# ysymyth/3D-SDN

Hardware: AMD Instinct MI355X
Metric: rendered-objects/sec (FFD decode + transform + silhouette/normal/depth @384, fwd+bwd) (higher is better)
Workload: dtype f32

## Files before the change

3d-sdn_amd/csrc/raster_fwd.hip:

```cpp
#include <mutex>
#include <type_traits>
#include <vector>

#include "camera_math.h"
#include "raster_math.h"
#include "sdn_common.h"

namespace sdn {

constexpr int TS = 32;
constexpr int NTHR = (TS / 2) * (TS / 2);
constexpr int NWAVE = NTHR / 64;
static_assert(NTHR % 64 == 0 && NTHR >= 2 * TS && TS <= 32, "tile / workgroup geometry (hit queue packs px, py in 5 bits)");
constexpr int QCAP = 512;
constexpr int FREC = 13;
#ifndef SDN_LAB_FLAT_MAX
#define SDN_LAB_FLAT_MAX 256
#endif
constexpr int FLAT_MAX = SDN_LAB_FLAT_MAX;
static_assert(FLAT_MAX >= 1 && FLAT_MAX <= 256, "a batch's stream holds at most 64 * 256 candidates: 14 bits of start, at most 256 passes (the marks are u16, 0xffff = none)");
#ifndef SDN_LAB_HIZ_MIN_LIST
#define SDN_LAB_HIZ_MIN_LIST 257
#endif
constexpr int HIZ_MIN_LIST = SDN_LAB_HIZ_MIN_LIST;
#ifndef SDN_K1_HIZ
#define SDN_K1_HIZ 1
#endif
constexpr uint32_t TB_CULLED = 0x000000FFu;

struct FwdParams {
    const float* faces;
    const float* textures;
    const float* bg;
    float* face_inv;
    int32_t* face_index_map;
    float* weight_map;
    float* depth_map;
    float* rgb_map;
    float* rgb_out;
    float* alpha_out;
    float* depth_out;
    const uint32_t* tilebox;
    const uint4* pixbox;
    const uint32_t* tile_off;
    const uint32_t* tile_list;
    const uint32_t* overflow;
    const uint32_t* tile_order;
    const uint32_t* thin_count;
    const float4* thin_list;
    unsigned long long* counters;
    uint32_t list_cap;
    double eps;
    int ts, bs, nf, S, ntx, flags, bg_per_batch;
    int hiz;
    float near_le, far_f;
};

constexpr float THIN_MARGIN = 4.0f;

__device__ __forceinline__ float face_margin_px(const float f[9], int S)
{
    const float ex0 = f[3] - f[0], ey0 = f[4] - f[1];
    const float ex1 = f[6] - f[0], ey1 = f[7] - f[1];
    const float ex2 = f[6] - f[3], ey2 = f[7] - f[4];
    const float l0 = sqrtf(ex0 * ex0 + ey0 * ey0);
    const float l1 = sqrtf(ex1 * ex1 + ey1 * ey1);
    const float l2 = sqrtf(ex2 * ex2 + ey2 * ey2);
    const float lmax = fmaxf(l0, fmaxf(l1, l2));
    const float perim = l0 + l1 + l2;
    float cmax = fmaxf(fmaxf(fabsf(f[0]), fabsf(f[1])), fmaxf(fabsf(f[3]), fabsf(f[4])));
    cmax = fmaxf(cmax, fmaxf(fabsf(f[6]), fabsf(f[7])));
    const float area2 = fabsf(ex0 * ey1 - ex1 * ey0) - 9.5367432e-7f * lmax * lmax;
    if (!(area2 > 0.0f)) return -1.0f;
    const float delta = 9.5367432e-7f * (1.0f + cmax);
    const float base = 0.004f * fmaxf(1.0f, (float)S * (1.0f / 1024.0f)) + 0.5f * (float)S * delta;
    const float m = base + 0.5f * (float)S * (delta * perim * lmax / area2);
    if (!(m < (float)S)) return -1.0f;
    return m;
}

constexpr int HIST_MAX = 4096;

template <bool K1, bool GATHER>
__global__ __launch_bounds__(256) void k_face_setup(const float* __restrict__ faces, int nf, int S, int ntx,
                                                     float* __restrict__ face_inv, uint32_t* __restrict__ tilebox,
                                                     uint4* __restrict__ pixbox, uint32_t* __restrict__ tile_count,
                                                     uint32_t* __restrict__ thin_count, float4* __restrict__ thin_list,
                                                     const FaceSource G)
{
    __shared__ uint32_t hist[HIST_MAX];
    const int ntiles = ntx * ntx;
    const bool use_lds = ntiles <= HIST_MAX;
    if (use_lds)
        for (int t = threadIdx.x; t < ntiles; t += 256) hist[t] = 0u;
    __syncthreads();
    const int b = blockIdx.y;
    const int t_local = blockIdx.x * 256 + threadIdx.x;
    uint32_t* gcount = tile_count + (size_t)b * ntiles;
    const bool pairs = GATHER && G.fill_back != 0;
    const int nthr = pairs ? G.nf0 : nf;
    float v[3][3], pf[9];
    if constexpr (GATHER) {
        if (t_local < nthr) {
            const int32_t* idx = G.faces_idx + (size_t)b * G.fstride + (size_t)t_local * 3;
#pragma unroll
            for (int k = 0; k < 3; k++) {
                const float* p = G.verts + ((size_t)b * G.nv + idx[k]) * 3;
                v[k][0] = G.flip_x ? p[0] * -1.0f : p[0];
                v[k][1] = p[1];
                v[k][2] = p[2];
            }
            Basis B;
            if (G.mode != 0) B = camera_basis(G.mode, G.eye, G.dir, G.up, b);
            const float wv = G.width ? G.width[b] : 1.0f;
#pragma unroll
            for (int k = 0; k < 3; k++) {
                float o[3];
                project_vertex(v[k], G.mode, B, G.width != nullptr, wv, o);
                pf[3 * k + 0] = o[0];
                pf[3 * k + 1] = o[1];
                pf[3 * k + 2] = o[2];
            }
        }
    }
    if (t_local < nthr)
    for (int rep = 0; rep < (pairs ? 2 : 1); rep++) {
    const int fn_local = t_local + (rep ? G.nf0 : 0);
    const long i = (long)b * nf + fn_local;
    float f[9];
    float nrm[3] = {0.f, 0.f, 0.f};
    if constexpr (GATHER) {
        if (G.normals_out) {
            if (rep)
                face_normal(v[2], v[1], v[0], G.sx, nrm);
            else
                face_normal(v[0], v[1], v[2], G.sx, nrm);
        }
#pragma unroll
        for (int k = 0; k < 3; k++)
#pragma unroll
            for (int d = 0; d < 3; d++) f[3 * k + d] = rep ? pf[3 * (2 - k) + d] : pf[3 * k + d];
    } else {
#pragma unroll
        for (int k = 0; k < 9; k++) f[k] = faces[i * 9 + k];
    }
    float inv[9] = {0, 0, 0, 0, 0, 0, 0, 0, 0};
    uint32_t tb = TB_CULLED;
    uint4 pb = make_uint4(0, 0, 0, 0);
    bool thin = false;
    if constexpr (K1) {
      if (!is_backface(f)) {
        bool finite = true;
// ... 134 lines not shown
            if (G.normals_out) {
                float* o = G.normals_out + i * 3;
                o[0] = nrm[0];
                o[1] = nrm[1];
                o[2] = nrm[2];
            }
        }
    }
    }
    __syncthreads();
    if (use_lds)
        for (int t = threadIdx.x; t < ntiles; t += 256) {
            const uint32_t c = hist[t];
            if (c) atomicAdd(&gcount[t], c);
        }
}

constexpr int ORDER_CLASSES = 64;
__device__ __forceinline__ int order_class(uint32_t entries, bool streams_all_faces)
{
    if (streams_all_faces) return 0;
    const int c = (int)(4.0f * __log2f((float)entries + 1.0f));
    return ORDER_CLASSES - 1 - min(ORDER_CLASSES - 1, c);
}

__global__ __launch_bounds__(256) void k_tile_offsets(const uint32_t* __restrict__ tile_count, int ntiles,
                                                       uint32_t list_cap, uint32_t* __restrict__ tile_off,
                                                       uint32_t* __restrict__ overflow, uint32_t* __restrict__ order_hist)
{
    __shared__ uint32_t wave_tot[4];
    __shared__ uint32_t carry_s;
    __shared__ uint32_t hist[ORDER_CLASSES];
    const int b = blockIdx.x, tid = threadIdx.x;
    if (tid < ORDER_CLASSES) hist[tid] = 0u;
    const uint32_t* cnt = tile_count + (size_t)b * ntiles;
    uint32_t* off = tile_off + (size_t)b * (ntiles + 1);
    if (tid == 0) carry_s = 0u;
    __syncthreads();
    for (int base = 0; base < ntiles; base += 256) {
        const int t = base + tid;
        const uint32_t v = t < ntiles ? cnt[t] : 0u;
        uint32_t incl = v;
#pragma unroll
        for (int d = 1; d < 64; d <<= 1) {
            const uint32_t o = __shfl_up(incl, d, 64);
            if ((tid & 63) >= d) incl += o;
        }
        if ((tid & 63) == 63) wave_tot[tid >> 6] = incl;
        __syncthreads();
        uint32_t wave_off = 0, total = 0;
#pragma unroll
        for (int w = 0; w < 4; w++) {
            const uint32_t x = wave_tot[w];
            if (w < (tid >> 6)) wave_off += x;
            total += x;
        }
        const uint32_t carry = carry_s;
        if (t < ntiles) off[t] = carry + wave_off + incl - v;
        __syncthreads();
        if (tid == 0) carry_s = carry + total;
        __syncthreads();
    }
    if (tid == 0) {
        off[ntiles] = carry_s;
        overflow[b] = carry_s > list_cap ? 1u : 0u;
    }
    const bool streams = carry_s > list_cap;
    for (int t = tid; t < ntiles; t += 256) atomicAdd(&hist[order_class(cnt[t], streams)], 1u);
    __syncthreads();
    if (tid < ORDER_CLASSES && hist[tid]) atomicAdd(&order_hist[tid], hist[tid]);
}

__global__ __launch_bounds__(256) void k_tile_order(const uint32_t* __restrict__ tile_count, int ntiles, int total,
                                                     const uint32_t* __restrict__ overflow,
                                                     const uint32_t* __restrict__ order_hist,
                                                     uint32_t* __restrict__ order_cursor, uint32_t* __restrict__ tile_order)
{
    __shared__ uint32_t base[ORDER_CLASSES];
    const int tid = threadIdx.x;
    if (tid < 64) {
        const uint32_t v = order_hist[tid];
        uint32_t incl = v;
#pragma unroll
        for (int d = 1; d < 64; d <<= 1) {
            const uint32_t o = __shfl_up(incl, d, 64);
            if (tid >= d) incl += o;
        }
        base[tid] = incl - v;
    }
    __shared__ uint32_t lcnt[ORDER_CLASSES], lbase[ORDER_CLASSES];
    if (tid < ORDER_CLASSES) lcnt[tid] = 0u;
    __syncthreads();
    const int g = blockIdx.x * 256 + tid;
    int c = 0;
    uint32_t local = 0;
    if (g < total) {
        c = order_class(tile_count[g], overflow[g / ntiles] != 0u);
        local = atomicAdd(&lcnt[c], 1u);
    }
    __syncthreads();
    if (tid < ORDER_CLASSES && lcnt[tid]) lbase[tid] = base[tid] + atomicAdd(&order_cursor[tid], lcnt[tid]);
    __syncthreads();
    if (g < total) tile_order[lbase[c] + local] = (uint32_t)g;
}

__global__ __launch_bounds__(256) void k_tile_fill(const uint32_t* __restrict__ tilebox, int nf, int ntx,
                                                    const uint32_t* __restrict__ tile_off,
                                                    const uint32_t* __restrict__ overflow, uint32_t list_cap,
                                                    uint32_t* __restrict__ tile_cursor, uint32_t* __restrict__ tile_list)
{
    __shared__ uint32_t cnt[HIST_MAX];
    __shared__ uint32_t base[HIST_MAX];
    const int b = blockIdx.y;
    if (overflow[b]) return;
    const int fn = blockIdx.x * 256 + threadIdx.x;
    const uint32_t v = fn < nf ? tilebox[(size_t)b * nf + fn] : TB_CULLED;
    const int tx0 = (int)(v & 255u), tx1 = (int)((v >> 8) & 255u), ty0 = (int)((v >> 16) & 255u), ty1 = (int)(v >> 24);
    const bool active = tx0 <= tx1;
    const int ntiles = ntx * ntx;
    const uint32_t* off = tile_off + (size_t)b * (ntiles + 1);
    uint32_t* cur = tile_cursor + (size_t)b * ntiles;
    uint32_t* lst = tile_list + (size_t)b * list_cap;
    if (ntiles > HIST_MAX) {
        if (active)
            for (int ty = ty0; ty <= ty1; ty++)
                for (int tx = tx0; tx <= tx1; tx++) {
                    const int tt = ty * ntx + tx;
                    lst[off[tt] + atomicAdd(&cur[tt], 1u)] = (uint32_t)fn;
                }
        return;
    }
    for (int t = threadIdx.x; t < ntiles; t += 256) cnt[t] = 0u;
    __syncthreads();
    if (active)
        for (int ty = ty0; ty <= ty1; ty++)
            for (int tx = tx0; tx <= tx1; tx++) atomicAdd(&cnt[ty * ntx + tx], 1u);
    __syncthreads();
    for (int t = threadIdx.x; t < ntiles; t += 256) {
        const uint32_t c = cnt[t];
        if (c) {
            base[t] = off[t] + atomicAdd(&cur[t], c);
            cnt[t] = 0u;
        }
    }
    __syncthreads();
    if (active)
        for (int ty = ty0; ty <= ty1; ty++)
            for (int tx = tx0; tx <= tx1; tx++) {
                const int tt = ty * ntx + tx;
                lst[base[tt] + atomicAdd(&cnt[tt], 1u)] = (uint32_t)fn;
            }
}

struct PixelResult {
    int fn;
    float w[3];
    float zp;
    float rgb[3];
    float alpha;
};

__device__ __forceinline__ PixelResult shade_pixel(const FwdParams& P, int b, unsigned long long key, int gx, int gy)
{
    PixelResult r;
    const bool want_rgb = (P.flags & SDN_RGB) != 0;
    float bgc[3] = {0.f, 0.f, 0.f};
    if (want_rgb) {
        const float* c = P.bg + (P.bg_per_batch ? 3 * b : 0);
        bgc[0] = c[0];
        bgc[1] = c[1];
        bgc[2] = c[2];
    }
    if (key == ~0ull) {
        r.fn = -1;
        r.w[0] = r.w[1] = r.w[2] = 0.0f;
        r.zp = P.far_f;
        r.alpha = 0.0f;
#pragma unroll
        for (int k = 0; k < 3; k++) r.rgb[k] = 0.0f * 0.0f + (1.0f - 0.0f) * bgc[k];
        return r;
    }
    const int fn = (int)(uint32_t)(key & 0xffffffffull);
    const size_t fidx = (size_t)b * P.nf + fn;
    float inv[9], f[9];
#pragma unroll
    for (int k = 0; k < 9; k++) inv[k] = P.face_inv[fidx * 9 + k];
#pragma unroll
    for (int k = 0; k < 9; k++) f[k] = P.faces[fidx * 9 + k];
    r.fn = fn;
    if (P.flags & SDN_K1_COVERAGE) {
        int pi[3];
        k1_order(f, pi);
        float inv_s[9], ws[3];
#pragma unroll
        for (int l = 0; l < 3; l++)
#pragma unroll
            for (int k = 0; k < 3; k++) inv_s[3 * l + k] = pi[l] == 0 ? inv[k] : (pi[l] == 1 ? inv[3 + k] : inv[6 + k]);
        bary_weights(inv_s, gx, gy, ws);
#pragma unroll
        for (int l = 0; l < 3; l++) {
            if (pi[l] == 0) r.w[0] = ws[l];
            if (pi[l] == 1) r.w[1] = ws[l];
            if (pi[l] == 2) r.w[2] = ws[l];
        }
    } else {
        bary_weights(inv, gx, gy, r.w);
    }
    r.zp = ord_unbits((uint32_t)(key >> 32));
    r.alpha = 1.0f;
    r.rgb[0] = r.rgb[1] = r.rgb[2] = 0.0f;
    if (want_rgb) {
        const bool face_color = (P.flags & SDN_FACE_COLOR) != 0;
        const int ts = face_color ? 2 : P.ts;
        const TexCoord tc = texture_coord(r.w, r.zp, f[2], f[5], f[8], ts, P.eps);
        const float* tex = face_color ? (P.textures + fidx * 3) : (P.textures + fidx * (size_t)ts * ts * ts * 3);
        float acc[3] = {0.f, 0.f, 0.f};
#pragma unroll
        for (int pn = 0; pn < 8; pn++) {
            int isc;
            float wgt;
            texture_corner(tc, pn, ts, isc, wgt);
            const float* t = face_color ? tex : (tex + (long)isc * 3);
#pragma unroll
            for (int k = 0; k < 3; k++) acc[k] = acc[k] + wgt * t[k];
        }
#pragma unroll
        for (int k = 0; k < 3; k++) r.rgb[k] = acc[k] * 1.0f + (1.0f - 1.0f) * bgc[k];
    }
    return r;
}

__device__ __forceinline__ void tile_epilogue(const FwdParams& P, const int b, const int X0, const int Y0,
                                              const unsigned long long* zbuf, const int tid)
{
    const int S = P.S;
    const bool aa = (P.flags & SDN_AA) != 0;
    const bool save = (P.flags & SDN_SAVE_MAPS) != 0;
    const bool lazy = (P.flags & SDN_LAZY_MAPS) != 0;
    const bool want_rgb = (P.flags & SDN_RGB) != 0;
    const bool want_alpha = (P.flags & SDN_ALPHA) != 0;
    const bool want_depth = (P.flags & SDN_DEPTH) != 0;
    const int qx = tid % (TS / 2), qy = tid / (TS / 2);
    const int R = aa ? S / 2 : S;
    float s_alpha = 0.f, s_depth = 0.f, s_rgb[3] = {0.f, 0.f, 0.f};
    bool any_valid = false;
#pragma unroll
    for (int dyi = 0; dyi < 2; dyi++) {
#pragma unroll
        for (int dx = 0; dx < 2; dx++) {
            const int dy = 1 - dyi;
            const int px = 2 * qx + dx, py = 2 * qy + dy;
            const int gx = X0 + px, gy = Y0 + py;
            if (gx >= S || gy >= S) continue;
            any_valid = true;
            const PixelResult r = shade_pixel(P, b, zbuf[py * TS + px], gx, gy);
            const size_t q = ((size_t)b * S + gy) * S + gx;
            if (save) {
                P.face_index_map[q] = r.fn;
                P.depth_map[q] = r.zp;
            }
            if (save && !lazy) {
                P.weight_map[q * 3 + 0] = r.w[0];
                P.weight_map[q * 3 + 1] = r.w[1];
                P.weight_map[q * 3 + 2] = r.w[2];
                if (want_rgb) {
                    P.rgb_map[q * 3 + 0] = r.rgb[0];
                    P.rgb_map[q * 3 + 1] = r.rgb[1];
                    P.rgb_map[q * 3 + 2] = r.rgb[2];
                }
            }
            if (aa) {
                s_alpha = s_alpha + r.alpha;
                s_depth = s_depth + r.zp;
#pragma unroll
                for (int k = 0; k < 3; k++) s_rgb[k] = s_rgb[k] + r.rgb[k];
            } else {
                const size_t o = ((size_t)b * S + (S - 1 - gy)) * S + gx;
                if (want_alpha) P.alpha_out[o] = r.alpha;
                if (want_depth) P.depth_out[o] = r.zp;
                if (want_rgb) {
#pragma unroll
                    for (int k = 0; k < 3; k++)
                        P.rgb_out[(((size_t)b * 3 + k) * S + (S - 1 - gy)) * S + gx] = r.rgb[k];
                }
            }
        }
    }
    if (aa && any_valid) {
        const int oc = X0 / 2 + qx;
        const int orow = R - 1 - (Y0 / 2 + qy);
        const size_t o = ((size_t)b * R + orow) * R + oc;
        if (want_alpha) P.alpha_out[o] = s_alpha * 0.25f;
        if (want_depth) P.depth_out[o] = s_depth * 0.25f;
        if (want_rgb) {
#pragma unroll
            for (int k = 0; k < 3; k++) P.rgb_out[(((size_t)b * 3 + k) * R + orow) * R + oc] = s_rgb[k] * 0.25f;
        }
    }
}

__device__ __forceinline__ void hiz_refresh(const uint32_t* zhi, uint32_t* blockmax, const int lane)
{
    uint32_t m[4] = {0u, 0u, 0u, 0u};
#pragma unroll
    for (int i = 0; i < 16; i++) m[i >> 2] = max(m[i >> 2], zhi[2 * (i * 64 + lane) + 1]);
#pragma unroll
// ... 639 lines not shown
}

__global__ __launch_bounds__(NTHR) void k_raster_tiles_k1_plain(const FwdParams P)
{
    __shared__ unsigned long long zbuf[TS * TS];
    __shared__ uint32_t next_batch;
    const int tid = threadIdx.x;
    const int lane = tid & 63;
    const int ntiles = P.ntx * P.ntx;
    const uint32_t gid = P.tile_order[blockIdx.x];
    const int b = (int)(gid / (uint32_t)ntiles), tile = (int)(gid % (uint32_t)ntiles);
    const int tx = tile % P.ntx, ty = tile / P.ntx;
    const int X0 = tx * TS, Y0 = ty * TS;
    const int S = P.S, nf = P.nf;
    for (int i = tid; i < TS * TS; i += NTHR) zbuf[i] = ~0ull;
    if (tid == 0) next_batch = 0;
    __syncthreads();
    const uint4* pbx = P.pixbox + (size_t)b * nf;
    const uint32_t* tb = P.tilebox + (size_t)b * nf;
    const float* faces_b = P.faces + (size_t)b * nf * 9;
    const float* finv_b = P.face_inv + (size_t)b * nf * 9;
    const uint32_t* zhi = reinterpret_cast<const uint32_t*>(zbuf);
    auto k1_pixel = [&](const float (&inv_s)[9], const float (&zs)[3], const uint32_t fn, const int xi, const int yi) {
        const float zmin = fminf(zs[0], fminf(zs[1], zs[2]));
        if (zmin > 0.0f && ord_bits(zmin * 0.99999f) > zhi[2 * ((yi - Y0) * TS + (xi - X0)) + 1]) return;
        float w[3];
        bary_weights(inv_s, xi, yi, w);
        const float zp = persp_depth(w, zs[0], zs[1], zs[2]);
        if (zp > P.near_le && zp < P.far_f) {
            const unsigned long long key = ((unsigned long long)ord_bits(zp) << 32) | fn;
            atomicMin(&zbuf[(yi - Y0) * TS + (xi - X0)], key);
        }
    };
    auto sorted_rows = [&](const K1Face& K, const float (&f)[9], const float (&inv)[9], float (&inv_s)[9], float (&zs)[3]) {
#pragma unroll
        for (int l = 0; l < 3; l++) {
            const int k = K.pi[l];
            zs[l] = k == 0 ? f[2] : (k == 1 ? f[5] : f[8]);
#pragma unroll
            for (int c = 0; c < 3; c++) inv_s[3 * l + c] = k == 0 ? inv[c] : (k == 1 ? inv[3 + c] : inv[6 + c]);
        }
    };
    constexpr int K1_SMALL = 32;
    auto raster_batch = [&](const bool have, const uint32_t fn) {
        float f[9], inv[9];
#pragma unroll
        for (int k = 0; k < 9; k++) f[k] = inv[k] = 0.0f;
        uint4 pb = make_uint4(0u, 0u, 0u, 0u);
        if (have) {
#pragma unroll
            for (int k = 0; k < 9; k++) f[k] = faces_b[(size_t)fn * 9 + k];
#pragma unroll
            for (int k = 0; k < 9; k++) inv[k] = finv_b[(size_t)fn * 9 + k];
            pb = pbx[fn];
        }
        const int lx0 = max((int)(pb.x & 0xffffu), X0), lx1 = min((int)(pb.x >> 16), X0 + TS - 1);
        const int ly0 = max((int)(pb.y & 0xffffu), Y0), ly1 = min((int)(pb.y >> 16), Y0 + TS - 1);
        const int lw = lx1 - lx0 + 1, lh = ly1 - ly0 + 1;
        const int area = (have && lw > 0 && lh > 0) ? lw * lh : 0;
        if (area > 0 && area <= K1_SMALL) {
            const K1Face K = k1_setup(f, S);
            float inv_s[9], zs[3];
            sorted_rows(K, f, inv, inv_s, zs);
            for (int xi = lx0; xi <= lx1; xi++) {
                int ya, yb;
                k1_column(K, xi, S, ya, yb);
                for (int yi = max(ya, ly0); yi <= min(yb, ly1); yi++) k1_pixel(inv_s, zs, fn, xi, yi);
            }
        }
        unsigned long long big = __ballot(area > K1_SMALL);
        while (big) {
            const int j = __builtin_amdgcn_readfirstlane(__ffsll((long long)big) - 1);
            big &= big - 1ull;
            float g[9], ginv[9];
#pragma unroll
            for (int k = 0; k < 9; k++) {
                g[k] = __int_as_float(__builtin_amdgcn_readlane(__float_as_int(f[k]), j));
                ginv[k] = __int_as_float(__builtin_amdgcn_readlane(__float_as_int(inv[k]), j));
            }
            const int x0 = __builtin_amdgcn_readlane(lx0, j), y0 = __builtin_amdgcn_readlane(ly0, j);
            const int w = __builtin_amdgcn_readlane(lw, j), h = __builtin_amdgcn_readlane(lh, j);
            const uint32_t gfn = (uint32_t)__builtin_amdgcn_readlane((int)fn, j);
            const K1Face K = k1_setup(g, S);
            float inv_s[9], zs[3];
            sorted_rows(K, g, ginv, inv_s, zs);
            const int col = lane >> 1;
            if (col < w) {
                int ya, yb;
                k1_column(K, x0 + col, S, ya, yb);
                ya = max(ya, y0);
                yb = min(yb, y0 + h - 1);
                for (int yi = ya + (lane & 1); yi <= yb; yi += 2) k1_pixel(inv_s, zs, gfn, x0 + col, yi);
            }
        }
    };
    if (P.overflow[b] == 0u) {
        const uint32_t* off = P.tile_off + (size_t)b * (ntiles + 1);
        const uint32_t lo = off[tile], hi = off[tile + 1];
        const uint32_t* lst = P.tile_list + (size_t)b * P.list_cap + lo;
        const int n_list = (int)(hi - lo);
        for (;;) {
            int base = 0;
            if (lane == 0) base = (int)atomicAdd(&next_batch, 64u);
            base = __builtin_amdgcn_readfirstlane(base);
            if (base >= n_list) break;
            const bool have = base + lane < n_list;
            raster_batch(have, have ? lst[base + lane] : 0u);
        }
    } else {
        for (int base = 0; base < nf; base += NTHR) {
            const int fn = base + tid;
            bool have = false;
            if (fn < nf) {
                const uint32_t v = tb[fn];
                have = (uint32_t)tx >= (v & 255u) && (uint32_t)tx <= ((v >> 8) & 255u) && (uint32_t)ty >= ((v >> 16) & 255u) &&
                       (uint32_t)ty <= (v >> 24);
            }
            raster_batch(have, (uint32_t)fn);
        }
    }
    __syncthreads();
    tile_epilogue(P, b, X0, Y0, zbuf, tid);
}

}

using namespace sdn;

struct FwdWorkspace {
    size_t tilebox, pixbox, zeroed, tile_count, tile_cursor, overflow, thin_count, counters, order_hist, zeroed_bytes,
        tile_order, tile_off, tile_list, thin_list, total;
    uint32_t list_cap;
    int ntx, ntiles;
};

static size_t align256(size_t n) { return (n + 255) & ~(size_t)255; }

static FwdWorkspace workspace_layout(int bs, int nf, int S)
{
    FwdWorkspace w;
    const size_t n = (size_t)bs * nf;
    w.ntx = (S + TS - 1) / TS;
    w.ntiles = w.ntx * w.ntx;
    w.list_cap = (uint32_t)(8 * (size_t)nf + 4 * (size_t)w.ntiles);
    size_t o = 0;
    w.tilebox = o;
    o += align256(n * sizeof(uint32_t));
    w.pixbox = o;
    o += align256(n * sizeof(uint4));
    w.zeroed = o;
    w.tile_count = o;
    o += align256((size_t)bs * w.ntiles * sizeof(uint32_t));
    w.tile_cursor = o;
    o += align256((size_t)bs * w.ntiles * sizeof(uint32_t));
    w.overflow = o;
    o += align256((size_t)bs * sizeof(uint32_t));
    w.thin_count = o;
    o += align256((size_t)bs * sizeof(uint32_t));
    w.counters = o;
    o += align256(16 * sizeof(unsigned long long));
    w.order_hist = o;
    o += align256(2 * ORDER_CLASSES * sizeof(uint32_t));
    w.zeroed_bytes = o - w.zeroed;
    w.tile_order = o;
    o += align256((size_t)bs * w.ntiles * sizeof(uint32_t));
    w.tile_off = o;
    o += align256((size_t)bs * (w.ntiles + 1) * sizeof(uint32_t));
    w.tile_list = o;
    o += align256((size_t)bs * w.list_cap * sizeof(uint32_t));
    w.thin_list = o;
    o += align256(n * 2 * sizeof(float4));
    w.total = o;
    return w;
}

SDN_API int sdn_raster_workspace_bytes(int bs, int nf, int S, size_t* out)
{
    if (bs <= 0 || nf <= 0 || S <= 0 || !out) return fail(SDN_EINVAL, "sdn_raster_workspace_bytes: bad sizes");
    *out = workspace_layout(bs, nf, S).total;
    return SDN_OK;
}

namespace sdn {
int rasterize_fwd_core(const FaceSource* src, const float* faces, const float* textures, int ts, int bs, int nf, int S, double near,
                       double far, double eps, const float* bg, int bg_per_batch, int flags, float* face_inv,
                       int32_t* face_index_map, float* weight_map, float* depth_map, float* rgb_map,
                       float* rgb_out, float* alpha_out, float* depth_out, void* workspace,
                       size_t workspace_bytes, sdnStream stream)
{
    if (!(flags & (SDN_RGB | SDN_ALPHA | SDN_DEPTH)))
        return fail(SDN_EINVAL, "sdn_rasterize_fwd: nothing to draw (rasterize.py:25-27)");
    if (!faces || !face_inv || bs <= 0 || nf <= 0 || S <= 0) return fail(SDN_EINVAL, "sdn_rasterize_fwd: bad faces/sizes");
    if (S > TS * 256) return fail(SDN_EINVAL, "sdn_rasterize_fwd: internal size %d > %d", S, TS * 256);
    if ((flags & SDN_AA) && (S & 1)) return fail(SDN_EINVAL, "sdn_rasterize_fwd: SDN_AA needs an even internal size");
    if (flags & SDN_RGB) {
        if (!textures || !bg || !rgb_out) return fail(SDN_EINVAL, "sdn_rasterize_fwd: rgb needs textures, bg, rgb_out");
        if (!(flags & SDN_FACE_COLOR) && ts < 2) return fail(SDN_EINVAL, "sdn_rasterize_fwd: texture size < 2");
    }
    if ((flags & SDN_ALPHA) && !alpha_out) return fail(SDN_EINVAL, "sdn_rasterize_fwd: alpha_out is NULL");
    if ((flags & SDN_DEPTH) && !depth_out) return fail(SDN_EINVAL, "sdn_rasterize_fwd: depth_out is NULL");
    if ((flags & SDN_SAVE_MAPS) && (!face_index_map || !depth_map))
        return fail(SDN_EINVAL, "sdn_rasterize_fwd: SDN_SAVE_MAPS needs the state maps");
    if ((flags & SDN_SAVE_MAPS) && !(flags & SDN_LAZY_MAPS) && (!weight_map || ((flags & SDN_RGB) && !rgb_map)))
        return fail(SDN_EINVAL, "sdn_rasterize_fwd: SDN_SAVE_MAPS needs the state maps");
    const FwdWorkspace W = workspace_layout(bs, nf, S);
    if (!workspace || workspace_bytes < W.total)
        return fail(SDN_ENOMEM, "sdn_rasterize_fwd: workspace %zu < %zu bytes", workspace_bytes, W.total);

    hipStream_t st = (hipStream_t)stream;
    char* ws = (char*)workspace;
    uint32_t* tilebox = (uint32_t*)(ws + W.tilebox);
    uint4* pixbox = (uint4*)(ws + W.pixbox);
    uint32_t* tile_count = (uint32_t*)(ws + W.tile_count);
    uint32_t* tile_cursor = (uint32_t*)(ws + W.tile_cursor);
    uint32_t* overflow = (uint32_t*)(ws + W.overflow);
    uint32_t* tile_off = (uint32_t*)(ws + W.tile_off);
    uint32_t* tile_list = (uint32_t*)(ws + W.tile_list);
    uint32_t* thin_count = (uint32_t*)(ws + W.thin_count);
    float4* thin_list = (float4*)(ws + W.thin_list);
    const int ntx = W.ntx;
    hipError_t me = hipMemsetAsync(ws + W.zeroed, 0, W.zeroed_bytes, st);
    if (me != hipSuccess) return fail(SDN_ELAUNCH, "hipMemsetAsync(tile counters): %s", hipGetErrorString(me));
    const dim3 face_grid(cdiv(nf, 256), bs);
    if (src && nf != (src->fill_back ? 2 : 1) * src->nf0) return fail(SDN_EINVAL, "rasterize_fwd_core: nf %d does not match the face source (%d faces, fill_back %d)", nf, src->nf0, src->fill_back);
    const dim3 setup_grid(cdiv((src && src->fill_back) ? src->nf0 : nf, 256), bs);
    const int k1 = (flags & SDN_K1_COVERAGE) ? 1 : 0;
    FaceSource G = FaceSource();
    if (src) G = *src;
#define SDN_FACE_SETUP(K1_, GATHER_)                                                                                          \
    hipLaunchKernelGGL((k_face_setup<K1_, GATHER_>), setup_grid, dim3(256), 0, st, faces, nf, S, ntx, face_inv, tilebox, pixbox, \
                       tile_count, thin_count, thin_list, G)
    if (k1 && src) SDN_FACE_SETUP(true, true);
    else if (k1) SDN_FACE_SETUP(true, false);
    else if (src) SDN_FACE_SETUP(false, true);
    else SDN_FACE_SETUP(false, false);
#undef SDN_FACE_SETUP
    int rc = check_launch("k_face_setup");
    if (rc) return rc;
    const uint32_t list_cap = (flags & SDN_STREAM_FACES) ? 0u : W.list_cap;
    uint32_t* order_hist = (uint32_t*)(ws + W.order_hist);
    uint32_t* tile_order = (uint32_t*)(ws + W.tile_order);
    hipLaunchKernelGGL(k_tile_offsets, dim3(bs), dim3(256), 0, st, tile_count, W.ntiles, list_cap, tile_off, overflow,
                       order_hist);
    if ((rc = check_launch("k_tile_offsets"))) return rc;
    hipLaunchKernelGGL(k_tile_order, dim3(cdiv(bs * W.ntiles, 256)), dim3(256), 0, st, tile_count, W.ntiles, bs * W.ntiles,
                       overflow, order_hist, order_hist + ORDER_CLASSES, tile_order);
    if ((rc = check_launch("k_tile_order"))) return rc;
    hipLaunchKernelGGL(k_tile_fill, face_grid, dim3(256), 0, st, tilebox, nf, ntx, tile_off, overflow, W.list_cap,
                       tile_cursor, tile_list);
    if ((rc = check_launch("k_tile_fill"))) return rc;

    FwdParams P;
    P.faces = faces;
    P.textures = textures;
    P.bg = bg;
    P.face_inv = face_inv;
    P.face_index_map = face_index_map;
    P.weight_map = weight_map;
    P.depth_map = depth_map;
    P.rgb_map = rgb_map;
    P.rgb_out = rgb_out;
    P.alpha_out = alpha_out;
    P.depth_out = depth_out;
    P.tilebox = tilebox;
    P.pixbox = pixbox;
    P.tile_off = tile_off;
    P.tile_list = tile_list;
    P.overflow = overflow;
    P.tile_order = tile_order;
    P.thin_count = thin_count;
    P.thin_list = thin_list;
    P.counters = (unsigned long long*)(ws + W.counters);
    P.list_cap = W.list_cap;
    P.eps = eps;
    P.ts = ts;
    P.bs = bs;
    P.nf = nf;
    P.S = S;
    P.ntx = ntx;
    P.flags = flags;
    P.bg_per_batch = bg_per_batch;
    float near_le = (float)near;
    if ((double)near_le > near) near_le = nextafterf(near_le, -INFINITY);
    P.near_le = near_le;
    P.far_f = (float)far;
    static const int hiz = [] { const char* e = getenv("SDN_RASTER_HIZ"); return e && e[0] >= '0' && e[0] <= '2' ? e[0] - '0' : 2; }();
    P.hiz = hiz;
    if (k1) {
        if (flags & SDN_COUNT_WORK) return fail(SDN_EINVAL, "sdn_rasterize_fwd: SDN_COUNT_WORK is not built for SDN_K1_COVERAGE");
        TimedLaunch timed(TIME_RASTER_TILES_K1, st, 0.0);
        static const bool plain = [] { const char* e = getenv("SDN_K1_PLAIN"); return e && e[0] == '1'; }();
        if (plain)
            hipLaunchKernelGGL(k_raster_tiles_k1_plain, dim3(ntx * ntx * bs), dim3(NTHR), 0, st, P);
        else
            hipLaunchKernelGGL(k_raster_tiles_k1, dim3(ntx * ntx * bs), dim3(NTHR), 0, st, P);
        return check_launch("k_raster_tiles_k1");
    }
    const dim3 grid(ntx * ntx * bs);
    if (flags & SDN_COUNT_WORK) {
        if (hiz == 0)
            hipLaunchKernelGGL((k_raster_tiles<true, 0>), grid, dim3(NTHR), 0, st, P);
        else if (hiz == 1)
            hipLaunchKernelGGL((k_raster_tiles<true, 1>), grid, dim3(NTHR), 0, st, P);
        else
            hipLaunchKernelGGL((k_raster_tiles<true, 2>), grid, dim3(NTHR), 0, st, P);
    } else {
        TimedLaunch timed(TIME_RASTER_TILES, st, 0.0);
        if (hiz == 0)
            hipLaunchKernelGGL((k_raster_tiles<false, 0>), grid, dim3(NTHR), 0, st, P);
        else if (hiz == 1)
            hipLaunchKernelGGL((k_raster_tiles<false, 1>), grid, dim3(NTHR), 0, st, P);
        else
            hipLaunchKernelGGL((k_raster_tiles<false, 2>), grid, dim3(NTHR), 0, st, P);
    }
    return check_launch("k_raster_tiles");
}
}

SDN_API int sdn_rasterize_fwd(const float* faces, const float* textures, int ts, int bs, int nf, int S, double near,
                              double far, double eps, const float* bg, int bg_per_batch, int flags, float* face_inv,
                              int32_t* face_index_map, float* weight_map, float* depth_map, float* rgb_map,
                              float* rgb_out, float* alpha_out, float* depth_out, void* workspace,
                              size_t workspace_bytes, sdnStream stream)
{
    return rasterize_fwd_core(nullptr, faces, textures, ts, bs, nf, S, near, far, eps, bg, bg_per_batch, flags, face_inv,
                              face_index_map, weight_map, depth_map, rgb_map, rgb_out, alpha_out, depth_out, workspace,
                              workspace_bytes, stream);
}

__global__ __launch_bounds__(256) void k_reshade_maps(const FwdParams P, long npx)
{
    const long q = (long)blockIdx.x * 256 + threadIdx.x;
    if (q >= npx) return;
    const int S = P.S;
    const int gx = (int)(q % S), gy = (int)((q / S) % S), b = (int)(q / ((long)S * S));
    const int fn = P.face_index_map[q];
    const unsigned long long key = fn < 0 ? ~0ull : (((unsigned long long)ord_bits(P.depth_map[q]) << 32) | (uint32_t)fn);
    const PixelResult r = shade_pixel(P, b, key, gx, gy);
    P.weight_map[q * 3 + 0] = r.w[0];
    P.weight_map[q * 3 + 1] = r.w[1];
    P.weight_map[q * 3 + 2] = r.w[2];
    if ((P.flags & SDN_RGB) && P.rgb_map) {
        P.rgb_map[q * 3 + 0] = r.rgb[0];
        P.rgb_map[q * 3 + 1] = r.rgb[1];
        P.rgb_map[q * 3 + 2] = r.rgb[2];
    }
}

namespace sdn {
int launch_reshade_maps(const float* faces, const float* textures, int ts, int bs, int nf, int S, double far, double eps,
                        const float* bg, int bg_per_batch, int flags, const float* face_inv, const int32_t* face_index_map,
                        const float* depth_map, float* weight_map, float* rgb_map, hipStream_t st)
{
    if (!faces || !face_inv || !face_index_map || !depth_map || !weight_map) return fail(SDN_EINVAL, "reshade: null pointer");
    if ((flags & SDN_RGB) && (!textures || !bg || !rgb_map)) return fail(SDN_EINVAL, "reshade: colour maps need textures, bg, rgb_map");
    FwdParams P = {};
    P.faces = faces;
    P.textures = textures;
    P.bg = bg;
    P.face_inv = const_cast<float*>(face_inv);
    P.face_index_map = const_cast<int32_t*>(face_index_map);
    P.depth_map = const_cast<float*>(depth_map);
    P.weight_map = weight_map;
    P.rgb_map = rgb_map;
    P.eps = eps;
    P.ts = ts;
    P.bs = bs;
    P.nf = nf;
    P.S = S;
    P.flags = flags;
    P.bg_per_batch = bg_per_batch;
    P.far_f = (float)far;
    const long npx = (long)bs * S * S;
    hipLaunchKernelGGL(k_reshade_maps, dim3(cdiv(npx, 256)), dim3(256), 0, st, P, npx);
    return check_launch("k_reshade_maps");
}
}

SDN_API int sdn_raster_work_counters(const void* workspace, int bs, int nf, int S, unsigned long long* out3, sdnStream stream)
{
    if (!workspace || !out3 || bs <= 0 || nf <= 0 || S <= 0) return fail(SDN_EINVAL, "sdn_raster_work_counters: bad arguments");
    const FwdWorkspace W = workspace_layout(bs, nf, S);
    hipStream_t st = (hipStream_t)stream;
    if (hipMemcpyAsync(out3, (const char*)workspace + W.counters, 3 * sizeof(unsigned long long), hipMemcpyDeviceToHost, st) !=
            hipSuccess ||
        hipStreamSynchronize(st) != hipSuccess)
        return fail(SDN_ELAUNCH, "sdn_raster_work_counters: copy failed");
    return SDN_OK;
}

SDN_API int sdn_raster_phase_clocks(const void* workspace, int bs, int nf, int S, unsigned long long* out8, sdnStream stream)
{
    if (!workspace || !out8 || bs <= 0 || nf <= 0 || S <= 0) return fail(SDN_EINVAL, "sdn_raster_phase_clocks: bad arguments");
    const FwdWorkspace W = workspace_layout(bs, nf, S);
    hipStream_t st = (hipStream_t)stream;
    if (hipMemcpyAsync(out8, (const char*)workspace + W.counters + 3 * sizeof(unsigned long long), 8 * sizeof(unsigned long long),
                       hipMemcpyDeviceToHost, st) != hipSuccess ||
        hipStreamSynchronize(st) != hipSuccess)
        return fail(SDN_ELAUNCH, "sdn_raster_phase_clocks: copy failed");
    return SDN_OK;
}
```

Baseline: 24490.

## Fuse tile offsets, tile ordering and tile fill into one binning kernel

Replaces the three-kernel binning chain (per-object prefix sum, tile-order classification, face-to-tile fill) with one launch. Extra blocks compute the tile ordering by class. The face blocks each redo the per-object prefix scan locally and process several faces per thread, with faces split into two halves that fill each tile's list from the front and the back using a second cursor array. The goal is to cut launch overhead and serial dependencies between the small kernels, at the cost of redundant prefix-scan work per block, doubled cursor workspace, and more LDS use.

```diff
diff --git a/3d-sdn_amd/csrc/raster_fwd.hip b/3d-sdn_amd/csrc/raster_fwd.hip
--- a/3d-sdn_amd/csrc/raster_fwd.hip
+++ b/3d-sdn_amd/csrc/raster_fwd.hip
@@ -1,3 +1,4 @@
+#include <algorithm>
 #include <mutex>
 #include <type_traits>
 #include <vector>
@@ -438,6 +439,171 @@
             }
 }
 
+#ifndef SDN_LAB_BIN_FPT
+#define SDN_LAB_BIN_FPT 4
+#endif
+constexpr int BIN_FPT = SDN_LAB_BIN_FPT;
+#ifndef SDN_LAB_BIN_TWO_ENDS
+#define SDN_LAB_BIN_TWO_ENDS 1
+#endif
+constexpr bool BIN_TWO_ENDS = SDN_LAB_BIN_TWO_ENDS != 0;
+constexpr int ORDER_BLOCKS_MAX = 32;
+constexpr int ORDER_CHUNK_MIN = 1024;
+
+__device__ __forceinline__ uint32_t object_total(const uint32_t* __restrict__ cnt, int ntiles, int lane)
+{
+    uint32_t s = 0;
+#pragma unroll 4
+    for (int t = lane; t < ntiles; t += 64) s += cnt[t];
+#pragma unroll
+    for (int d = 32; d >= 1; d >>= 1) s += __shfl_xor(s, d, 64);
+    return s;
+}
+
+template <int FPT>
+__global__ __launch_bounds__(256) void k_tile_bin(const uint32_t* __restrict__ tilebox, int nf, int ntx, int bs, int nfb, int nob,
+                                                   int chunk, const uint32_t* __restrict__ tile_count, uint32_t list_cap,
+                                                   uint32_t list_stride, uint32_t* __restrict__ tile_off,
+                                                   uint32_t* __restrict__ overflow, uint32_t* __restrict__ tile_cursor,
+                                                   uint32_t* __restrict__ tile_list, uint32_t* __restrict__ tile_order)
+{
+    extern __shared__ uint32_t bin_lds[];
+    __shared__ uint32_t wave_tot[4];
+    __shared__ uint32_t cbase[ORDER_CLASSES];
+    const int tid = threadIdx.x, lane = tid & 63, wave = tid >> 6;
+    const int ntiles = ntx * ntx;
+    if ((int)blockIdx.x < nob) {
+        const int k = blockIdx.x;
+        const int total = bs * ntiles;
+        for (int i = tid; i < nob * ORDER_CLASSES; i += 256) bin_lds[i] = 0u;
+        __syncthreads();
+        for (int b = wave; b < bs; b += 4) {
+            const uint32_t* cnt = tile_count + (size_t)b * ntiles;
+            const bool streams = object_total(cnt, ntiles, lane) > list_cap;
+#pragma unroll 4
+            for (int t = lane; t < ntiles; t += 64) {
+                const int c = order_class(streams ? 0u : cnt[t], streams);
+                atomicAdd(&bin_lds[((b * ntiles + t) / chunk) * ORDER_CLASSES + c], 1u);
+            }
+        }
+        __syncthreads();
+        if (tid < 64) {
+            uint32_t all = 0, before = 0;
+            for (int j = 0; j < nob; j++) {
+                const uint32_t x = bin_lds[j * ORDER_CLASSES + tid];
+                all += x;
+                if (j < k) before += x;
+            }
+            uint32_t incl = all;
+#pragma unroll
+            for (int d = 1; d < 64; d <<= 1) {
+                const uint32_t o = __shfl_up(incl, d, 64);
+                if (tid >= d) incl += o;
+            }
+            cbase[tid] = incl - all + before;
+        }
+        __syncthreads();
+        const int g0 = k * chunk, g1 = min(total, g0 + chunk);
+        if (g0 >= g1) return;
+        for (int b = g0 / ntiles + wave; b <= (g1 - 1) / ntiles; b += 4) {
+            const uint32_t* cnt = tile_count + (size_t)b * ntiles;
+            const bool streams = object_total(cnt, ntiles, lane) > list_cap;
+            const int t0 = max(g0 - b * ntiles, 0), t1 = min(g1 - b * ntiles, ntiles);
+            for (int t = t0 + lane; t < t1; t += 64) {
+                const int c = order_class(streams ? 0u : cnt[t], streams);
+                tile_order[atomicAdd(&cbase[c], 1u)] = (uint32_t)(b * ntiles + t);
+            }
+        }
+        return;
+    }
+    const int blk = (int)blockIdx.x - nob;
+    const int b = blk / nfb, fb = blk - b * nfb;
+    uint32_t* cnt = bin_lds;
+    uint32_t* base = bin_lds + ntiles;
+    const uint32_t* gcnt = tile_count + (size_t)b * ntiles;
+    const int split = (nf + 1) / 2, nfb_front = (split + 256 * FPT - 1) / (256 * FPT);
+    const bool back = BIN_TWO_ENDS && fb >= nfb_front;
+    const int fn0 = (back ? split + (fb - nfb_front) * (256 * FPT) : fb * (256 * FPT)) + tid;
+    const int fn_end = (BIN_TWO_ENDS && !back) ? split : nf;
+    uint32_t v[FPT];
+#pragma unroll
+    for (int j = 0; j < FPT; j++) {
+        const int fn = fn0 + j * 256;
+        v[j] = fn < fn_end ? tilebox[(size_t)b * nf + fn] : TB_CULLED;
+    }
+    for (int t = tid; t < ntiles; t += 256) {
+        base[t] = gcnt[t];
+        cnt[t] = 0u;
+    }
+    __syncthreads();
+    const int run = (ntiles + 255) / 256;
+    const int r0 = min(tid * run, ntiles), r1 = min(r0 + run, ntiles);
+    uint32_t s = 0;
+    for (int t = r0; t < r1; t++) s += base[t];
+    uint32_t incl = s;
+#pragma unroll
+    for (int d = 1; d < 64; d <<= 1) {
+        const uint32_t o = __shfl_up(incl, d, 64);
+        if (lane >= d) incl += o;
+    }
+    if (lane == 63) wave_tot[wave] = incl;
+    __syncthreads();
+    uint32_t acc = incl - s, total = 0;
+#pragma unroll
+    for (int w = 0; w < 4; w++) {
+        const uint32_t x = wave_tot[w];
+        if (w < wave) acc += x;
+        total += x;
+    }
+    for (int t = r0; t < r1; t++) {
+        const uint32_t x = base[t];
+        base[t] = acc;
+        acc += x;
+    }
+    __syncthreads();
+    const bool over = total > list_cap;
+    if (fb == 0) {
+        uint32_t* off = tile_off + (size_t)b * (ntiles + 1);
+        for (int t = tid; t < ntiles; t += 256) off[t] = base[t];
+        if (tid == 0) {
+            off[ntiles] = total;
+            overflow[b] = over ? 1u : 0u;
+        }
+    }
+    if (over) return;
+    uint32_t* cur = tile_cursor + (size_t)b * ntiles;
+    uint32_t* lst = tile_list + (size_t)b * list_stride;
+#pragma unroll
+    for (int j = 0; j < FPT; j++) {
+        const int tx0 = (int)(v[j] & 255u), tx1 = (int)((v[j] >> 8) & 255u), ty0 = (int)((v[j] >> 16) & 255u), ty1 = (int)(v[j] >> 24);
+        if (tx0 <= tx1)
+            for (int ty = ty0; ty <= ty1; ty++)
+                for (int tx = tx0; tx <= tx1; tx++) atomicAdd(&cnt[ty * ntx + tx], 1u);
+    }
+    __syncthreads();
+    for (int t = tid; t < ntiles; t += 256) {
+        const uint32_t c = cnt[t];
+        if (c) {
+            if (back)
+                base[t] += gcnt[t] - c - atomicAdd(&cur[(size_t)bs * ntiles + t], c);
+            else
+                base[t] += atomicAdd(&cur[t], c);
+            cnt[t] = 0u;
+        }
+    }
+    __syncthreads();
+#pragma unroll
+    for (int j = 0; j < FPT; j++) {
+        const int tx0 = (int)(v[j] & 255u), tx1 = (int)((v[j] >> 8) & 255u), ty0 = (int)((v[j] >> 16) & 255u), ty1 = (int)(v[j] >> 24);
+        if (tx0 <= tx1)
+            for (int ty = ty0; ty <= ty1; ty++)
+                for (int tx = tx0; tx <= tx1; tx++) {
+                    const int tt = ty * ntx + tx;
+                    lst[base[tt] + atomicAdd(&cnt[tt], 1u)] = (uint32_t)(fn0 + j * 256);
+                }
+    }
+}
+
 struct PixelResult {
     int fn;
     float w[3];
@@ -1383,7 +1549,7 @@
     w.tile_count = o;
     o += align256((size_t)bs * w.ntiles * sizeof(uint32_t));
     w.tile_cursor = o;
-    o += align256((size_t)bs * w.ntiles * sizeof(uint32_t));
+    o += align256(2 * (size_t)bs * w.ntiles * sizeof(uint32_t));
     w.overflow = o;
     o += align256((size_t)bs * sizeof(uint32_t));
     w.thin_count = o;
@@ -1471,15 +1637,32 @@
     const uint32_t list_cap = (flags & SDN_STREAM_FACES) ? 0u : W.list_cap;
     uint32_t* order_hist = (uint32_t*)(ws + W.order_hist);
     uint32_t* tile_order = (uint32_t*)(ws + W.tile_order);
-    hipLaunchKernelGGL(k_tile_offsets, dim3(bs), dim3(256), 0, st, tile_count, W.ntiles, list_cap, tile_off, overflow,
-                       order_hist);
-    if ((rc = check_launch("k_tile_offsets"))) return rc;
-    hipLaunchKernelGGL(k_tile_order, dim3(cdiv(bs * W.ntiles, 256)), dim3(256), 0, st, tile_count, W.ntiles, bs * W.ntiles,
-                       overflow, order_hist, order_hist + ORDER_CLASSES, tile_order);
-    if ((rc = check_launch("k_tile_order"))) return rc;
-    hipLaunchKernelGGL(k_tile_fill, face_grid, dim3(256), 0, st, tilebox, nf, ntx, tile_off, overflow, W.list_cap,
-                       tile_cursor, tile_list);
-    if ((rc = check_launch("k_tile_fill"))) return rc;
+    if (W.ntiles <= HIST_MAX) {
+        const int total = bs * W.ntiles;
+        int nob = std::min(ORDER_BLOCKS_MAX, (int)cdiv(total, ORDER_CHUNK_MIN));
+        const int chunk = (int)cdiv(total, nob);
+        nob = (int)cdiv(total, chunk);
+        const int split = (nf + 1) / 2;
+        const int nfb = BIN_TWO_ENDS ? (int)(cdiv(split, 256 * BIN_FPT) + cdiv(nf - split, 256 * BIN_FPT)) : (int)cdiv(nf, 256 * BIN_FPT);
+#ifdef SDN_LAB_BIN_LDS_TILES
+        const size_t lds = sizeof(uint32_t) * (size_t)std::max(2 * std::max(W.ntiles, SDN_LAB_BIN_LDS_TILES), nob * ORDER_CLASSES);
+#else
+        const size_t lds = sizeof(uint32_t) * (size_t)std::max(2 * W.ntiles, nob * ORDER_CLASSES);
+#endif
+        hipLaunchKernelGGL((k_tile_bin<BIN_FPT>), dim3(nob + bs * nfb), dim3(256), lds, st, tilebox, nf, ntx, bs, nfb, nob, chunk,
+                           tile_count, list_cap, W.list_cap, tile_off, overflow, tile_cursor, tile_list, tile_order);
+        if ((rc = check_launch("k_tile_bin"))) return rc;
+    } else {
+        hipLaunchKernelGGL(k_tile_offsets, dim3(bs), dim3(256), 0, st, tile_count, W.ntiles, list_cap, tile_off, overflow,
+                           order_hist);
+        if ((rc = check_launch("k_tile_offsets"))) return rc;
+        hipLaunchKernelGGL(k_tile_order, dim3(cdiv(bs * W.ntiles, 256)), dim3(256), 0, st, tile_count, W.ntiles, bs * W.ntiles,
+                           overflow, order_hist, order_hist + ORDER_CLASSES, tile_order);
+        if ((rc = check_launch("k_tile_order"))) return rc;
+        hipLaunchKernelGGL(k_tile_fill, face_grid, dim3(256), 0, st, tilebox, nf, ntx, tile_off, overflow, W.list_cap,
+                           tile_cursor, tile_list);
+        if ((rc = check_launch("k_tile_fill"))) return rc;
+    }
 
     FwdParams P;
     P.faces = faces;
```

Result: no change. 24640, median of 4 (+0.6%).
